# mcahny/vps

Hardware: AMD Instinct MI355X
Metric: frames/sec FuseTrack 1024x2048 (higher is better)
Workload: dtype f32-grade: f16x3 split operands (fp16 pair with scaled residual, 22 significand bits) on MFMA, f32 accumulate

## Files before the change

include/vps_hip.h:

```cpp
#ifndef VPS_HIP_H
#define VPS_HIP_H

#include <stdint.h>

#ifdef __cplusplus
extern "C" {
#endif

int vps_abi_version(void);
const char* vps_build_info(void);

enum { VPS_ACT_NONE = 0, VPS_ACT_RELU = 1, VPS_ACT_LEAKY = 2 };
enum { VPS_PREC_F32 = 0, VPS_PREC_BF16 = 1, VPS_PREC_BF16X3 = 2, VPS_PREC_BF16X6 = 3, VPS_PREC_F16X3 = 4 };

typedef struct vps_conv_desc {
    const float* in;
    int32_t N, H, W;
    int32_t in_ld;
    int32_t in_coff;
    int32_t cin_pad;
    const float* w;
    int32_t cout, cout_pad, kpad;
    int32_t KH, KW, stride;
    int32_t pad_y[2], pad_x[2];
// ... 2 lines not shown
    int32_t out_ld, out_coff;
    int32_t Qh, Qw;
    int32_t os_y, os_x;
    int32_t nclass;
    const float* scale;
    const float* shift;
    const float* res;
    int32_t res_ld, res_coff, res_shift;
    int32_t act;
    float slope;
    const float* offset;
    int32_t off_ld;
    int32_t tile_n;
    int32_t ksplit;
    float* ws;
    int32_t prec;
    const void* w_split;
    int32_t korder;
    int32_t* status;
    double* gn_stats;
    int32_t gn_cpg, gn_rep;
    int32_t* tile_counter;
    const void* w_thin;
} vps_conv_desc;

int vps_conv2d(const vps_conv_desc* d, void* stream);

typedef struct vps_tensor4 {
    float* p;
    int64_t sn, sc, sh, sw;
} vps_tensor4;

int vps_resample2d(vps_tensor4 in, vps_tensor4 flow, vps_tensor4 out,
                   int B, int C, int H, int W, void* stream);

int vps_channelnorm(vps_tensor4 in, vps_tensor4 out, int B, int C, int H, int W, void* stream);

int vps_correlation(const float* in1, int ld1, int coff1, const float* in2, int ld2, int coff2,
                    float* out, int out_ld, int out_coff,
                    int N, int H, int W, int C, int max_disp, int stride2,
                    int act, float slope, void* stream);
int vps_correlation_f16(const float* in1, int ld1, int coff1, const float* in2, int ld2, int coff2,
                        float* out, int out_ld, int out_coff, int N, int H, int W, int C,
                        int max_disp, int stride2, int act, float slope, int32_t* status, void* stream);

int vps_flow_warp(const float* in, int in_ld, int in_coff, const float* flow, int flow_ld, int flow_coff,
// ... 156 lines not shown
```

vps_amd/csrc/conv_mfma.hip:

```cpp
#include "conv_common.h"

namespace {
template <int TM, int TN, int WAVES_M, int WAVES_N, bool DEFORM>
__global__ __launch_bounds__(256, 2)
void conv_mfma_f32_kernel(const vps_conv_desc d, const int M, const int tiles_m, const int tiles_n,
                          const int ksteps_per_split) {
    constexpr int BN = WAVES_N * TN * 32;
    static_assert(WAVES_M * TM * 32 == BM, "block M tile must be 128");
    static_assert(WAVES_M * WAVES_N == 4, "4 wavefronts per block");
    constexpr int NB = BN / 32;

    __shared__ __attribute__((aligned(16))) float As[BM * LDS_LD];
    __shared__ __attribute__((aligned(16))) float Bs[BN * LDS_LD];

    const int t = threadIdx.x;
    int swz = xcd_swizzle(blockIdx.x, gridDim.x);
    int tile_n, tile_m, cls, split;
    decode_tile(d, swz, tiles_n, tiles_m, tile_n, tile_m, cls, split);

    const int py = cls / d.os_x, px = cls - py * d.os_x;
    const int pad_y = d.pad_y[py], pad_x = d.pad_x[px];
    const float* __restrict__ wcls = d.w + (size_t)cls * d.cout_pad * d.kpad;

    const int H = d.H, W = d.W, KH = d.KH, KW = d.KW, cin_pad = d.cin_pad;
// ... 710 lines not shown
            else hipLaunchKernelGGL((conv_mfma_bf16h_kernel<TM, TN, WAVES_M, WAVES_N, MODE, 2, 2>), grid, block, 0, s, d, p.tiles_m, p.tiles_n, p.chunks_per_split);
        });
        return;
    }
#define VPS_CONV_LAUNCH(KERNEL) hipLaunchKernelGGL((KERNEL), grid, block, 0, s, d, p.M, p.tiles_m, p.tiles_n, p.per_split)
    if (p.kernel == CONV_K_F32) {
        if (d.offset) VPS_CONV_LAUNCH((conv_mfma_f32_kernel<TM, TN, WAVES_M, WAVES_N, true>));
        else VPS_CONV_LAUNCH((conv_mfma_f32_kernel<TM, TN, WAVES_M, WAVES_N, false>));
        return;
    }
    const bool tapmajor = d.korder == 0 && d.KH * d.KW > 1;
    with_prec<true>(d.prec, [&](auto mode) {
        constexpr int MODE = decltype(mode)::value;
        if (d.offset) VPS_CONV_LAUNCH((conv_mfma_bf16p_kernel<TM, TN, WAVES_M, WAVES_N, MODE, false, true>));
        else if (tapmajor) VPS_CONV_LAUNCH((conv_mfma_bf16p_kernel<TM, TN, WAVES_M, WAVES_N, MODE, true>));
        else VPS_CONV_LAUNCH((conv_mfma_bf16p_kernel<TM, TN, WAVES_M, WAVES_N, MODE, false>));
    });
#undef VPS_CONV_LAUNCH
}

conv_switches conv_switches_now(const vps_conv_desc& d) {
    const auto on = [](const char* name) { const char* const e = getenv(name); return !(e && atoi(e) == 0); };
    const auto not0 = [](const char* name) { const char* const e = getenv(name); return !(e && e[0] == '0'); };
    static const bool s2_halo = not0("VPS_S2_HALO"), thin = on("VPS_THIN"), debug_occ = getenv("VPS_DEBUG_OCC") != nullptr;
    conv_switches sw = {true, true, true, true, s2_halo, thin, debug_occ};
    if (d.prec != VPS_PREC_F16X3) return sw;
    if (d.tile_n == 32) {
        if (d.cout > 16) sw.n32 = not0("VPS_N32");
        else if (d.nclass == 4) sw.n16t = on("VPS_N16T");
    } else if (d.tile_n <= 128 && d.KH == 1) sw.pw = on("VPS_PW");
    else if (d.tile_n == 128 && d.KH == 3 && d.stride == 1) sw.h8p = on("VPS_H8P");
    return sw;
}

const conv_limits& conv_limits_once(const bool debug) {
    static const conv_limits lim = [debug] {
        conv_limits l = {};
        int dev = 0;
        (void)hipGetDevice(&dev);
        (void)hipDeviceGetAttribute(&l.cus, hipDeviceAttributeMultiprocessorCount, dev);
        vpsi_conv_pw_limits(l, debug);
        vpsi_conv_thin_limits(l, debug);
        if (debug) vpsi_conv_q_debug_occ();
        return l;
    }();
    return lim;
}

}

extern "C" int vps_conv2d(const vps_conv_desc* dp, void* stream) {
    if (!dp) return VPS_EARG(1);
    const vps_conv_desc& d = *dp;
    if (const int e = vpsi_conv_check(d)) return e;
    const conv_switches sw = conv_switches_now(d);
    const conv_plan p = vpsi_conv_plan(d, conv_limits_once(sw.debug_occ), sw);
    hipStream_t s = (hipStream_t)stream;
    switch (p.kernel) {
        case CONV_K_NONE: return p.err;
        case CONV_K_SMALL3X3V: case CONV_K_SMALL_BATCHED: case CONV_K_SMALL: vpsi_launch_conv_small(d, p, s); break;
        case CONV_K_THIN: vpsi_launch_conv_thin(d, p, s); break;
        case CONV_K_DCN256:
            hipLaunchKernelGGL((conv_mfma_bf16p_kernel<2, 4, 2, 2, VPS_PREC_F16X3, false, true>), dim3(p.grid), dim3(p.block), 0, s, d, p.M, p.tiles_m, p.tiles_n, p.per_split);
            break;
        case CONV_K_N16T: case CONV_K_N32: case CONV_K_N16: vpsi_launch_conv_n16(d, p, s); break;
        case CONV_K_H8S2: vpsi_launch_conv_h8s2(d, p, s); break;
        case CONV_K_H8P: vpsi_launch_conv_h8p(d, p, s); break;
        case CONV_K_H8: vpsi_launch_conv_h8(d, p, s); break;
        case CONV_K_PW: vpsi_launch_conv_pw(d, p, s); break;
        case CONV_K_Q: vpsi_launch_conv_q(d, p, s); break;
        default:
            if (d.tile_n == 128) launch_conv<2, 2, 2, 2>(d, p, s);
            else if (d.tile_n == 64) launch_conv<2, 1, 2, 2>(d, p, s);
            else launch_conv<1, 1, 4, 1>(d, p, s);
    }
    int st = vps_launch_status();
    if (st || !p.needs_reduce) return st;
    const size_t total = (size_t)d.nclass * p.M * d.cout;
    if (p.reduce_v4) hipLaunchKernelGGL(conv_splitk_reduce_kernel<4>, dim3(stream_grid((long)(total / 4), 256)), dim3(256), 0, s, d, p.M);
    else hipLaunchKernelGGL(conv_splitk_reduce_kernel<1>, dim3(stream_grid((long)total, 256)), dim3(256), 0, s, d, p.M);
    return vps_launch_status();
}
```

vps_amd/csrc/conv_plan.cpp:

```cpp
#include "conv_plan.h"
#include <stdint.h>

namespace {

constexpr int BM = 128, BK = 32;

inline int cdiv(long a, long b) { return (int)((a + b - 1) / b); }
inline size_t in_bytes(const vps_conv_desc& d) { return (size_t)d.N * d.H * d.W * d.in_ld * sizeof(float); }
inline size_t out_bytes(const vps_conv_desc& d) { return (size_t)d.N * d.Ho * d.Wo * d.out_ld * sizeof(float); }
inline bool two_plane(int prec) { return prec == VPS_PREC_F16X3 || prec == VPS_PREC_BF16X3 || prec == VPS_PREC_BF16; }

constexpr int H8_MIN_CHUNKS = 3;
constexpr int PW_MIN_ROUNDS = 2;

conv_plan fail(conv_plan p, int n) { p.kernel = CONV_K_NONE; p.err = VPS_EARG(n); return p; }

conv_plan plan_small(const vps_conv_desc& d, conv_plan p) {
    p.block = 256;
    p.G = 1; p.logG = 0;
    while (p.G < 64 && p.G < (d.cin_pad >> 2)) { p.G <<= 1; ++p.logG; }
    const size_t wbytes = (size_t)(d.cout <= 2 ? 2 : 4) * d.kpad * sizeof(float);
    if (d.KH == 3 && d.KW == 3 && d.stride == 1 && d.nclass == 1 && d.pad_y[0] == 1 && d.pad_x[0] == 1 && d.Ho == d.H && d.Wo == d.W &&
        wbytes <= 150 * 1024 && (d.cout <= 2 || d.cout_pad >= 4) && in_bytes(d) < 0xFFFFFFF0ull &&
        (long)d.N * d.H * d.W < 0x7fffffffL) {
// ... 23 lines not shown
    long blocks = (waves + 3) / 4; if (blocks > 8192) blocks = 8192; if (blocks < 1) blocks = 1;
    p.kernel = CONV_K_SMALL; p.grid = (unsigned)blocks;
    return p;
}

bool plan_thin(const vps_conv_desc& d, const conv_limits& lim, const conv_switches& sw, conv_plan& p) {
    if (!sw.thin || !d.w_thin || d.prec != VPS_PREC_F16X3 || d.offset || d.res || d.nclass != 1 || d.ksplit != 1 || d.korder != 0) return false;
    if (d.KH != d.KW || d.cout_pad != 64 || d.tile_n != 64 || (d.cout & 3) || ((uintptr_t)d.w_thin & 15)) return false;
    if (d.pad_y[0] != d.KH / 2 || d.pad_x[0] != d.KH / 2 || d.pad_y[1] != d.KH / 2 || d.pad_x[1] != d.KH / 2) return false;
    if (in_bytes(d) >= 0xFFFFFFF0ull) return false;
    if (((d.out_ld | d.out_coff) & 3) || ((uintptr_t)d.out & 15) || out_bytes(d) >= 0xFFFFFFF0ull) return false;
    int i = 0;
    while (i < 4 && !(d.KH == conv_thin_shapes[i].ks && d.stride == conv_thin_shapes[i].s && d.cin_pad == conv_thin_shapes[i].c4)) ++i;
    if (i == 4) return false;
    const int ph = conv_thin_shapes[i].ph;
    const int tiles_x = (d.Qw + 31) / 32, tiles_y = (d.Qh + ph - 1) / ph;
    const long ntiles = (long)d.N * tiles_x * tiles_y;
    if (ntiles < 512 || ntiles > 0x7fffffffL) return false;
    const int resident = (lim.thin_per_cu[i] > 0 ? lim.thin_per_cu[i] : 1) * (lim.cus > 0 ? lim.cus : 256);
    const long rounds = (ntiles + resident - 1) / resident;
    p.kernel = CONV_K_THIN; p.thin = i; p.tiles_n = tiles_x; p.tiles_m = tiles_y; p.ntiles = (int)ntiles;
    p.grid = (unsigned)((ntiles + rounds - 1) / rounds); p.block = 256;
    return true;
}

bool plan_pw(const vps_conv_desc& d, const conv_limits& lim, const conv_switches& sw, conv_plan& p) {
    if (!sw.pw || d.prec != VPS_PREC_F16X3 || d.offset || d.KH != 1 || d.KW != 1 || d.nclass != 1 || d.ksplit != 1 || d.gn_stats) return false;
    if (d.pad_y[0] || d.pad_x[0] || (d.cin_pad & 31) || d.kpad != d.cin_pad || (d.tile_n != 128 && d.tile_n != 64)) return false;
    const int nk = d.kpad / BK;
    if (nk < 2 || (nk & 1)) return false;
    if (d.Ho != d.Qh || d.Wo != d.Qw || (d.stride == 1 && (d.H != d.Qh || d.W != d.Qw))) return false;
    if (((d.cout | d.out_ld | d.out_coff) & 3) || ((uintptr_t)d.out & 15) || out_bytes(d) >= 0xFFFFFE00ull) return false;
    if (d.res && (((d.res_ld | d.res_coff) & 3) || ((uintptr_t)d.res & 15) || d.res_shift < 0 || d.res_shift > 4 ||
                  (size_t)d.N * (d.Ho >> d.res_shift) * (d.Wo >> d.res_shift) * d.res_ld * sizeof(float) >= 0xFFFFFE00ull)) return false;
    if (in_bytes(d) >= 0xFFFFFE00ull) return false;
    const int per_cu = lim.pw_per_cu[d.tile_n == 128 ? 1 : 0];
    const int resident = (per_cu > 0 ? per_cu : 1) * (lim.cus > 0 ? lim.cus : 256);
    const long total = (long)p.tiles_m * p.tiles_n;
    const int unit = 8 * p.tiles_n;
    if (resident < unit || total < (long)PW_MIN_ROUNDS * resident) return false;
    const long rounds = (total + resident - 1) / resident;
    long grid = (total + rounds - 1) / rounds;
    grid = (grid + unit - 1) / unit * unit;
    if (grid > resident) grid = resident / unit * unit;
    const int mper = (int)(grid / unit);
    p.kernel = CONV_K_PW; p.grid = (unsigned)grid; p.nk = nk; p.nit = (p.tiles_m + mper * 8 - 1) / (mper * 8);
    return true;
}

}

const conv_thin_shape conv_thin_shapes[4] = {{8, 3, 1, 8}, {12, 3, 1, 8}, {4, 7, 2, 8}, {12, 7, 2, 4}};

const char* vpsi_conv_kernel_name(int kernel) {
    static const char* const names[] = {"none", "small3x3v", "small_batched", "small", "thin", "dcn256", "n16t", "n32", "n16",
                                        "h8s2", "h8p", "h8", "halo", "pw", "q", "f32", "bf16p"};
    return kernel >= 0 && kernel <= CONV_K_BF16P ? names[kernel] : "?";
}

int vpsi_conv_check(const vps_conv_desc& d) {
    if (!d.in || !d.out) return VPS_EARG(2);
    if (d.prec < VPS_PREC_F32 || d.prec > VPS_PREC_F16X3) return VPS_EARG(12);
    if (d.prec == VPS_PREC_F32 ? !d.w : !d.w_split) return VPS_EARG(13);
    if ((d.in_ld & 3) || (d.in_coff & 3) || (d.cin_pad & 3) || d.cin_pad <= 0) return VPS_EARG(3);
    if ((d.kpad % BK) || d.kpad < d.KH * d.KW * d.cin_pad || (d.korder != 0 && d.korder != 1)) return VPS_EARG(4);
    if (d.korder == 1 && d.kpad != d.KH * d.KW * ((d.cin_pad + BK - 1) / BK) * BK) return VPS_EARG(14);
    if (d.tile_n != 32 && d.tile_n != 64 && d.tile_n != 128 && !(d.tile_n == 256 && d.offset && d.prec == VPS_PREC_F16X3 && d.korder == 1)) return VPS_EARG(5);
    if (d.cout_pad % d.tile_n || d.cout > d.cout_pad || d.cout <= 0) return VPS_EARG(6);
    if (d.nclass != d.os_y * d.os_x || d.nclass < 1 || d.os_y > 2 || d.os_x > 2) return VPS_EARG(7);
    if (d.ksplit < 1 || (d.ksplit > 1 && !d.ws)) return VPS_EARG(8);
    if (d.offset && (d.nclass != 1 || d.off_ld < 2 * d.KH * d.KW || d.KH * d.KW > 9 || d.H > 65535 || d.W > 65535)) return VPS_EARG(9);
    if (d.offset && d.prec != VPS_PREC_F32 && d.korder != 1) return VPS_EARG(17);
    if (((uintptr_t)d.in & 15) || ((uintptr_t)d.w & 15) || ((uintptr_t)d.w_split & 15)) return VPS_EARG(10);
    if (d.prec != VPS_PREC_F32 && in_bytes(d) >= 0xFFFFFFF0ull) return VPS_EARG(16);
    if (d.gn_stats && (!d.offset || d.prec == VPS_PREC_F32 || d.ksplit != 1 || d.gn_rep < 1 || (d.gn_rep & (d.gn_rep - 1)) || (d.gn_cpg != 4 && (d.gn_cpg < 8 || (d.gn_cpg & 7))) || d.cout % d.gn_cpg ||
                       ((d.cout | d.out_ld | d.out_coff) & 3) || ((uintptr_t)d.out & 15) || d.res || ((uintptr_t)d.gn_stats & 7)))
        return VPS_EARG(15);
    const long Ml = (long)d.N * d.Qh * d.Qw;
    if (Ml <= 0 || Ml > 0x7fffffffL) return VPS_EARG(11);
    return 0;
}

conv_plan vpsi_conv_plan(const vps_conv_desc& d, const conv_limits& lim, const conv_switches& sw) {
    conv_plan p = {};
    const int M = p.M = (int)((long)d.N * d.Qh * d.Qw);
    if (d.cout <= 4 && d.prec == VPS_PREC_F32 && !d.offset && d.ksplit == 1 && d.tile_n == 32) return plan_small(d, p);
    if (plan_thin(d, lim, sw, p)) return p;

    const int BN = d.tile_n;
    const int tiles_m = p.tiles_m = cdiv(M, BM);
    const int tiles_n = p.tiles_n = d.cout_pad / BN;
    const int ksteps = d.kpad / BK;
    p.block = 256;
    p.needs_reduce = d.ksplit > 1 && !d.tile_counter;
    if (BN == 256) {
        p.per_split = cdiv(ksteps, d.ksplit);
        if (cdiv(ksteps, p.per_split) != d.ksplit) return fail(p, 20);
        p.kernel = CONV_K_DCN256; p.grid = (unsigned)((long)tiles_m * tiles_n * d.ksplit); p.reduce_v4 = true;
        return p;
    }
    const int ntap = d.KH * d.KW;
    const int nch = d.korder == 1 ? ksteps / ntap : 0;
    const bool chunk_split = d.ksplit > 1 && d.korder == 1 && nch > 0 && cdiv(nch, cdiv(nch, d.ksplit)) == d.ksplit;
    const int per_split = p.per_split = chunk_split ? cdiv(nch, d.ksplit) * ntap : cdiv(ksteps, d.ksplit);
    p.chunks_per_split = per_split / ntap;
    if (cdiv(ksteps, per_split) != d.ksplit) return fail(p, 20);
    const long nblk = (long)tiles_m * tiles_n * d.nclass * d.ksplit;
    if (nblk <= 0 || nblk > 0x7fffffffL) return fail(p, 21);
    p.reduce_v4 = !((d.cout | d.cout_pad | d.out_ld | d.out_coff) & 3) && !((uintptr_t)d.out & 15) &&
                  (!d.res || (!((d.res_ld | d.res_coff) & 3) && !((uintptr_t)d.res & 15)));
// ... 39 lines not shown
```

vps_amd/csrc/conv_plan.h:

```cpp
#pragma once
#include <stddef.h>
#include "../../include/vps_hip.h"

#ifndef VPS_EARG
#define VPS_EARG(x) (-1000 - (x))
#endif

enum conv_kernel {
    CONV_K_NONE = 0,
    CONV_K_SMALL3X3V,
    CONV_K_SMALL_BATCHED,
    CONV_K_SMALL,
    CONV_K_THIN,
    CONV_K_DCN256,
    CONV_K_N16T,
    CONV_K_N32,
    CONV_K_N16,
    CONV_K_H8S2,
    CONV_K_H8P,
    CONV_K_H8,
    CONV_K_HALO,
    CONV_K_PW,
    CONV_K_Q,
    CONV_K_F32,
    CONV_K_BF16P,
};

struct conv_plan {
    int kernel;
    int err;
    int M;
    int tiles_m, tiles_n;
    int per_split;
    int chunks_per_split;
    unsigned grid, block;
    size_t smem;
    int nk, nit;
    int G, logG, nslot;
    int runs_per_row, total_runs;
    int thin;
    int ntiles;
    bool needs_reduce;
    bool reduce_v4;
};

struct conv_limits {
    int cus;
    int pw_per_cu[2];
    int thin_per_cu[4];
};

struct conv_switches {
    bool pw;
    bool h8p;
    bool n16t;
    bool n32;
    bool s2_halo;
    bool thin;
    bool debug_occ;
};

struct conv_thin_shape { int c4, ks, s, ph; };
extern const conv_thin_shape conv_thin_shapes[4];

int vpsi_conv_check(const vps_conv_desc& d);
conv_plan vpsi_conv_plan(const vps_conv_desc& d, const conv_limits& lim, const conv_switches& sw);
const char* vpsi_conv_kernel_name(int kernel);

#ifdef __HIPCC__
void vpsi_launch_conv_small(const vps_conv_desc& d, const conv_plan& p, hipStream_t s);
void vpsi_launch_conv_thin(const vps_conv_desc& d, const conv_plan& p, hipStream_t s);
void vpsi_launch_conv_n16(const vps_conv_desc& d, const conv_plan& p, hipStream_t s);
void vpsi_launch_conv_h8(const vps_conv_desc& d, const conv_plan& p, hipStream_t s);
void vpsi_launch_conv_h8p(const vps_conv_desc& d, const conv_plan& p, hipStream_t s);
void vpsi_launch_conv_h8s2(const vps_conv_desc& d, const conv_plan& p, hipStream_t s);
void vpsi_launch_conv_pw(const vps_conv_desc& d, const conv_plan& p, hipStream_t s);
void vpsi_launch_conv_q(const vps_conv_desc& d, const conv_plan& p, hipStream_t s);
void vpsi_conv_pw_limits(conv_limits& lim, bool debug);
void vpsi_conv_thin_limits(conv_limits& lim, bool debug);
void vpsi_conv_q_debug_occ();
#endif
```

vps_amd/csrc/info.hip:

```cpp
#include "common.h"

#define VPS_ABI_VERSION 19

extern "C" int vps_abi_version(void) { return VPS_ABI_VERSION; }

extern "C" const char* vps_build_info(void) {
#define VPS_STR2(x) #x
#define VPS_STR(x) VPS_STR2(x)
    return "libvpship abi=" VPS_STR(VPS_ABI_VERSION) " arch=gfx950 wave=64 mfma=f32_32x32x2,bf16_32x32x16(split x3/x6),f16_32x32x16(split x3) "
           "kernels=conv_mfma,flow_ops,nn_ops,det_ops,head_ops,pan_ops,post_ops,jpeg_ops";
}
```

vps_amd/flownet2.py:

```python
import torch
import torch.nn as nn

from . import hip, nhwc
from .base import HipModule


def _conv(cin, cout, k=3, stride=1):
    return nn.Sequential(nn.Conv2d(cin, cout, k, stride=stride, padding=(k - 1) // 2, bias=True), nn.LeakyReLU(0.1))


def _iconv(cin, cout):
    return nn.Sequential(nn.Conv2d(cin, cout, 3, padding=1, bias=True))


def _deconv(cin, cout):
    return nn.Sequential(nn.ConvTranspose2d(cin, cout, 4, 2, 1, bias=True), nn.LeakyReLU(0.1))


def _pred(cin):
    return nn.Conv2d(cin, 2, 3, padding=1, bias=True)


class _Net(nn.Module):

# ... 113 lines not shown
        self.conv1 = _conv(64, 64, stride=2); self.conv1_1 = _conv(64, 128)
        self.conv2 = _conv(128, 128, stride=2); self.conv2_1 = _conv(128, 128)
        self.conv3 = _conv(128, 256, stride=2); self.conv3_1 = _conv(256, 256)
        self.conv4 = _conv(256, 512, stride=2); self.conv4_1 = _conv(512, 512)
        self.conv5 = _conv(512, 512, stride=2); self.conv5_1 = _conv(512, 512)
        self.conv6 = _conv(512, 1024, stride=2); self.conv6_1 = _conv(1024, 1024)
        self.deconv5 = _deconv(1024, 512); self.deconv4 = _deconv(1026, 256)
        self.deconv3 = _deconv(770, 128); self.deconv2 = _deconv(386, 64)
        self.inter_conv5 = _iconv(1026, 512); self.inter_conv4 = _iconv(770, 256)
        self.inter_conv3 = _iconv(386, 128); self.inter_conv2 = _iconv(194, 64)
        self.predict_flow6 = _pred(1024); self.predict_flow5 = _pred(512); self.predict_flow4 = _pred(256)
        self.predict_flow3 = _pred(128); self.predict_flow2 = _pred(64)
        for n in ('6_to_5', '5_to_4', '4_to_3', '3_to_2'):
            setattr(self, 'upsampled_flow' + n, nn.ConvTranspose2d(2, 2, 4, 2, 1))

    def run(self, x6, ws, tag):
        p = self._p
        N, H, W = x6.N, x6.H, x6.W
        h2, w2 = H // 4, W // 4
        cat2 = ws.fmap(tag + 'cat2', N, h2, w2, 194)
        cat3 = ws.fmap(tag + 'cat3', N, h2 // 2, w2 // 2, 386)
        cat4 = ws.fmap(tag + 'cat4', N, h2 // 4, w2 // 4, 770)
        cat5 = ws.fmap(tag + 'cat5', N, h2 // 8, w2 // 8, 1026)
        c0 = p['conv0'](x6.window(0, 6), ws=ws, name=tag + 'c0', temp=True)
        t = p['conv1'](c0, ws=ws, name=tag + 'c1', temp=True)
        ws.release(c0)
        c1 = p['conv1_1'](t, ws=ws, name=tag + 'c11', temp=True)
        ws.release(t)
        t = p['conv2'](c1, ws=ws, name=tag + 'c2', temp=True)
        ws.release(c1)
        p['conv2_1'](t, out=cat2.window(0, 128), ws=ws)
        ws.release(t)
        t = p['conv3'](cat2.window(0, 128), ws=ws, name=tag + 'c3', temp=True)
        p['conv3_1'](t, out=cat3.window(0, 256), ws=ws)
        t = p['conv4'](cat3.window(0, 256), ws=ws, name=tag + 'c4', temp=True)
        p['conv4_1'](t, out=cat4.window(0, 512), ws=ws)
        t = p['conv5'](cat4.window(0, 512), ws=ws, name=tag + 'c5', temp=True)
        p['conv5_1'](t, out=cat5.window(0, 512), ws=ws)
        t = p['conv6'](cat5.window(0, 512), ws=ws, name=tag + 'c6', temp=True)
        c6 = p['conv6_1'](t, ws=ws, name=tag + 'c61', temp=True)
        flow = p['predict_flow6'](c6, ws=ws, name=tag + 'flow6')
        feat = c6
        for lvl, cat, enc_c, dec_c in ((5, cat5, 512, 512), (4, cat4, 512, 256), (3, cat3, 256, 128), (2, cat2, 128, 64)):
            p['upsampled_flow%d_to_%d' % (lvl + 1, lvl)](flow, out=cat.window(enc_c + dec_c, 2), ws=ws)
            p['deconv%d' % lvl](feat, out=cat.window(enc_c, dec_c), ws=ws)
            inter = p['inter_conv%d' % lvl](cat, ws=ws, name='%sinter%d' % (tag, lvl), temp=True)
            flow = p['predict_flow%d' % lvl](inter, ws=ws, name='%sflow%d' % (tag, lvl))
            ws.release(inter)
            feat = cat
        return flow


class FlowNetFusion(_Net):
    def __init__(self):
        super().__init__()
        self.conv0 = _conv(11, 64)
        self.conv1 = _conv(64, 64, stride=2); self.conv1_1 = _conv(64, 128)
        self.conv2 = _conv(128, 128, stride=2); self.conv2_1 = _conv(128, 128)
        self.deconv1 = _deconv(128, 32); self.deconv0 = _deconv(162, 16)
        self.inter_conv1 = _iconv(162, 32); self.inter_conv0 = _iconv(82, 16)
        self.predict_flow2 = _pred(128); self.predict_flow1 = _pred(32); self.predict_flow0 = _pred(16)
        self.upsampled_flow2_to_1 = nn.ConvTranspose2d(2, 2, 4, 2, 1)
        self.upsampled_flow1_to_0 = nn.ConvTranspose2d(2, 2, 4, 2, 1)

    def run(self, x11, ws, tag):
        p = self._p
        N, H, W = x11.N, x11.H, x11.W
        cat0 = ws.fmap(tag + 'cat0', N, H, W, 82)
        cat1 = ws.fmap(tag + 'cat1', N, H // 2, W // 2, 162)
        p['conv0'](x11, out=cat0.window(0, 64), ws=ws)
        t = p['conv1'](cat0.window(0, 64), ws=ws, name=tag + 'c1', temp=True)
        p['conv1_1'](t, out=cat1.window(0, 128), ws=ws)
        ws.release(t)
        t = p['conv2'](cat1.window(0, 128), ws=ws, name=tag + 'c2', temp=True)
        c2 = p['conv2_1'](t, ws=ws, name=tag + 'c21', temp=True)
        ws.release(t)
        flow2 = p['predict_flow2'](c2, ws=ws, name=tag + 'flow2')
        p['upsampled_flow2_to_1'](flow2, out=cat1.window(160, 2), ws=ws)
        p['deconv1'](c2, out=cat1.window(128, 32), ws=ws)
        ws.release(c2)
        inter1 = p['inter_conv1'](cat1, ws=ws, name=tag + 'inter1', temp=True)
        flow1 = p['predict_flow1'](inter1, ws=ws, name=tag + 'flow1')
        ws.release(inter1)
        p['upsampled_flow1_to_0'](flow1, out=cat0.window(80, 2), ws=ws)
        p['deconv0'](cat1, out=cat0.window(64, 16), ws=ws)
        inter0 = p['inter_conv0'](cat0, ws=ws, name=tag + 'inter0', temp=True)
        return p['predict_flow0'](inter0, ws=ws, name=tag + 'flow0', keep=True)


class FlowNet2(HipModule):

    def __init__(self, args=None, batchNorm=False, div_flow=20., requires_grad=False):
        super().__init__()
        assert not batchNorm
# ... 82 lines not shown
```

vps_amd/hip.py:

```python
import ctypes
import os
from ctypes import (POINTER, Structure, byref, c_char_p, c_double, c_float, c_int, c_int32, c_int64, c_uint64,
                    c_void_p)

import torch

_HERE = os.path.dirname(os.path.abspath(__file__))
LIB_PATH = os.environ.get('VPS_HIP_LIB') or os.path.join(_HERE, 'csrc', 'libvpship.so')
ABI_VERSION = 19

ACT_NONE, ACT_RELU, ACT_LEAKY = 0, 1, 2
PREC_F32, PREC_BF16, PREC_BF16X3, PREC_BF16X6, PREC_F16X3 = 0, 1, 2, 3, 4

SYMBOLS = [
    'vps_abi_version', 'vps_build_info', 'vps_conv2d', 'vps_resample2d', 'vps_channelnorm', 'vps_correlation',
    'vps_flow_warp', 'vps_nchw_to_nhwc', 'vps_nhwc_to_nchw', 'vps_resize', 'vps_pool3x3s2', 'vps_bfp_gather',
    'vps_bfp_scatter', 'vps_bfp_scatter_all', 'vps_axpb', 'vps_flow_prep', 'vps_flow_prep_pad', 'vps_flow_stage', 'vps_flow_stage_full', 'vps_groupnorm_relu', 'vps_groupnorm_apply', 'vps_tcea_temporal',
    'vps_tcea_modulate', 'vps_tcea_modulate_ld', 'vps_correlation_f16', 'vps_roi_align', 'vps_nms_batched', 'vps_delta2bbox', 'vps_bbox_overlaps',
    'vps_row_softmax', 'vps_mask_count', 'vps_mask_commit', 'vps_mask_removal', 'vps_mask_removal_dep', 'vps_mask_removal_hist', 'vps_frame_tail', 'vps_mask_level', 'vps_panoptic_combine',
    'vps_panoptic_combine_dev', 'vps_rpn_select', 'vps_rpn_collect', 'vps_maskroi_select', 'vps_maskroi_finish', 'vps_track_assign', 'vps_pan_instances',
    'vps_unify_hist', 'vps_unify_tables', 'vps_unify_write', 'vps_image_prep', 'vps_resize_u8', 'vps_segment_stats', 'vps_segment_paint', 'vps_pair_count',
    'vps_png_info', 'vps_png_decode_bgr8', 'vps_jpeg_info', 'vps_jpeg_decode_coef', 'vps_jpeg_reconstruct',
]


class ConvDesc(Structure):
    _fields_ = [
        ('inp', c_void_p), ('N', c_int32), ('H', c_int32), ('W', c_int32),
        ('in_ld', c_int32), ('in_coff', c_int32), ('cin_pad', c_int32),
        ('w', c_void_p), ('cout', c_int32), ('cout_pad', c_int32), ('kpad', c_int32),
        ('KH', c_int32), ('KW', c_int32), ('stride', c_int32),
        ('pad_y', c_int32 * 2), ('pad_x', c_int32 * 2),
        ('out', c_void_p), ('Ho', c_int32), ('Wo', c_int32), ('out_ld', c_int32), ('out_coff', c_int32),
        ('Qh', c_int32), ('Qw', c_int32), ('os_y', c_int32), ('os_x', c_int32), ('nclass', c_int32),
        ('scale', c_void_p), ('shift', c_void_p), ('res', c_void_p),
        ('res_ld', c_int32), ('res_coff', c_int32), ('res_shift', c_int32),
        ('act', c_int32), ('slope', c_float),
        ('offset', c_void_p), ('off_ld', c_int32),
        ('tile_n', c_int32), ('ksplit', c_int32), ('ws', c_void_p),
        ('prec', c_int32), ('w_split', c_void_p), ('korder', c_int32), ('status', c_void_p),
        ('gn_stats', c_void_p), ('gn_cpg', c_int32), ('gn_rep', c_int32), ('tile_counter', c_void_p), ('w_thin', c_void_p),
    ]


class Tensor4(Structure):
    _fields_ = [('p', c_void_p), ('sn', c_int64), ('sc', c_int64), ('sh', c_int64), ('sw', c_int64)]


class PanInst(Structure):
    _fields_ = [('sx0', c_int32), ('sy0', c_int32), ('sx1', c_int32), ('sy1', c_int32), ('seg_ch', c_int32),
                ('bx1', c_int32), ('by1', c_int32), ('bx2', c_int32), ('by2', c_int32), ('mask_idx', c_int32)]


_lib = None
_host = None


class VpsHipError(RuntimeError):
    pass


def csrc_sha16():
    import glob
    import hashlib
# ... 166 lines not shown
```

vps_amd/nhwc.py:

```python
import ctypes
import math
import os
import weakref
from ctypes import c_float, c_int, c_void_p

import torch

from . import hip


def _ceil(a, b):
    return (a + b - 1) // b * b


_PREC_NAMES = {'f32': hip.PREC_F32, 'bf16': hip.PREC_BF16, 'bf16x3': hip.PREC_BF16X3, 'bf16x6': hip.PREC_BF16X6, 'f16x3': hip.PREC_F16X3}
PREC_NAMES = _PREC_NAMES
_PLANES = {hip.PREC_BF16: 1, hip.PREC_BF16X3: 2, hip.PREC_BF16X6: 3, hip.PREC_F16X3: 3}
MFMA_PRODUCTS = {hip.PREC_F32: 1, hip.PREC_BF16: 1, hip.PREC_BF16X3: 3, hip.PREC_BF16X6: 6, hip.PREC_F16X3: 3}
F16_SLOTS = 4096
_F16_STATUS = {}
_F16_LAYERS = {}
_F16_NEXT = [1]
F16_FALLBACKS = [0]

# ... 491 lines not shown
                               '%d->%d k%dx%d s%d %s%s n%d %dx%d tile%d ksplit%d p%d' % (self.cin, self.cout, self.KH, self.KW, self.stride,
                                                                                   'T' if self.transposed else '', 'D' if self.deform else '',
                                                                                   x.N, x.H, x.W, tile_n, ksplit, self.prec),
                               self.bytes(x.N, x.H, x.W, res is not None)))
        else:
            hip.conv2d(d)
        if len(cache) >= 16:
            cache.clear()
        cache[ckey] = (d, wsb if ksplit > 1 else None, x.t, out.t, None if res is None else res.t, None if offset is None else offset.t)
        return out

    def bytes(self, x_N, x_H, x_W, has_res=False):
        Ho, Wo = self.out_hw(x_H, x_W)
        wbytes = self.nclass * self.cout * self.KH * self.KW * self.cin * (4 if self.prec == hip.PREC_F32 else 2 * _PLANES[self.prec])
        return 4.0 * x_N * (x_H * x_W * self.cin + Ho * Wo * self.cout * (2 if has_res else 1)) + wbytes

    def flops(self, x_N, x_H, x_W):
        if self.transposed:
            return 2.0 * x_N * x_H * x_W * 4 * self.cout * self.cin * self.KH * self.KW
        Ho, Wo = self.out_hw(x_H, x_W)
        return 2.0 * x_N * Ho * Wo * self.cout * self.cin * self.KH * self.KW


def pack_conv_module(m, bn=None, act=hip.ACT_NONE, slope=0.1, device='cuda', deform=False, prec=None):
    import torch.nn as nn
    bnd = None
    if bn is not None:
        bnd = dict(weight=bn.weight, bias=bn.bias, running_mean=bn.running_mean, running_var=bn.running_var, eps=bn.eps)
    if isinstance(m, nn.ConvTranspose2d):
        return PackedConv(m.weight, m.bias, bnd, stride=m.stride[0], padding=m.padding[0], act=act, slope=slope,
                          transposed=True, device=device, prec=prec)
    return PackedConv(m.weight, m.bias, bnd, stride=m.stride[0], padding=m.padding[0], act=act, slope=slope,
                      device=device, deform=deform, prec=prec)


def pack_linear(weight, bias, act=hip.ACT_NONE, device='cuda', chw=None, prec=None):
    w = weight.detach().float().cpu()
    if chw is not None:
        C, S = chw
        w = w.view(w.shape[0], C, S).permute(0, 2, 1).reshape(w.shape[0], C * S)
    return PackedConv(w.view(w.shape[0], w.shape[1], 1, 1), bias, None, 1, 0, act=act, device=device, prec=prec)


def resize(x, out, mode='bilinear', alpha=1.0):
    hip.check(hip.load().vps_resize(x.ptr(), x.ld, x.coff, x.H, x.W, out.ptr(), out.ld, out.coff, out.H, out.W,
                                    x.N, x.C, 0 if mode == 'bilinear' else 1, float(alpha), hip.stream_ptr()), 'vps_resize')
# ... 113 lines not shown
```

Baseline: 55.57.

## Fuse thin stride-1 conv0 into following stride-2 conv1 front kernel

```diff
diff --git a/include/vps_hip.h b/include/vps_hip.h
--- a/include/vps_hip.h
+++ b/include/vps_hip.h
@@ -48,6 +48,16 @@
     int32_t gn_cpg, gn_rep;
     int32_t* tile_counter;
     const void* w_thin;
+    const float* pre_in;
+    int32_t pre_in_ld, pre_in_coff, pre_cin_pad;
+    const void* pre_w_thin;
+    const float* pre_scale;
+    const float* pre_shift;
+    int32_t pre_act;
+    float pre_slope;
+    float* pre_out;
+    int32_t pre_out_ld, pre_out_coff;
+    int32_t* pre_status;
 } vps_conv_desc;
 
 int vps_conv2d(const vps_conv_desc* d, void* stream);
diff --git a/vps_amd/csrc/conv_front.hip b/vps_amd/csrc/conv_front.hip
--- /dev/null
+++ b/vps_amd/csrc/conv_front.hip
@@ -0,0 +1,254 @@
+#include "conv_common.h"
+
+namespace {
+
+constexpr int TMODE = VPS_PREC_F16X3;
+typedef _Float16 h16;
+typedef vec8<h16> h16x8;
+typedef vec4<h16> h16x4;
+
+struct FTap { int ph, j, i, idx; };
+constexpr FTap front_tap(int ts) {
+    int base = 0;
+    for (int ph = 0; ph < 4; ++ph) {
+        const int a = ph >> 1, b = ph & 1, J = 2 - a, I = 2 - b;
+        if (ts < base + J * I) {
+            const int t = ts - base, j = t / I, i = t - j * I;
+            return FTap{ph, j, i, (2 * j + a) * 3 + 2 * i + b};
+        }
+        base += J * I;
+    }
+    return FTap{0, 0, 0, 0};
+}
+template <int N, typename F>
+__device__ __forceinline__ void static_for(F&& f) {
+    if constexpr (N > 0) {
+        static_for<N - 1>(f);
+        f(std::integral_constant<int, N - 1>{});
+    }
+}
+
+template <int C4>
+struct FrontShape {
+    static constexpr int PH = 4, PW = 32;
+    static constexpr int TR = 2 * PH + 1, TC = 2 * PW + 1;
+    static constexpr int TPOS = TR * TC, NGRP = (TPOS + 31) / 32;
+    static constexpr int PR = TR + 2, PC = TC + 2, NPOS = PR * PC;
+    static constexpr int NV = C4 / 4;
+    static constexpr int NK16 = (3 * C4 + 15) / 16;
+    static constexpr int APLANE = NPOS * C4 + 16;
+    static constexpr int TWH = 3 * 2 * NK16 * 512;
+    static constexpr int SW = PW + 1;
+    static constexpr int TROWS = (2 * (PH + 1) + 2 * PH) * SW;
+    static constexpr int TPLANE = TROWS * LDS_LDH;
+    static constexpr int WBH = 8 * 512;
+    static constexpr size_t smem = (size_t)(2 * APLANE + TWH + 2 * TPLANE + 2 * WBH) * 2 + 128 * sizeof(float);
+    static_assert((2 * APLANE) % 8 == 0 && TWH % 8 == 0 && (2 * TPLANE) % 8 == 0, "16-byte aligned regions");
+    static_assert(smem <= 160 * 1024, "LDS budget of the CU");
+};
+
+template <int C4, bool STORE>
+__global__ __launch_bounds__(512, 1)
+void conv_front_kernel(const vps_conv_desc d, const int tiles_x, const int tiles_y) {
+    typedef FrontShape<C4> S;
+    typedef Split<TMODE> SM;
+    constexpr int PH = S::PH, PW = S::PW, TC = S::TC, TPOS = S::TPOS, NGRP = S::NGRP, PC = S::PC, NPOS = S::NPOS, NV = S::NV, NK16 = S::NK16;
+    constexpr int APLANE = S::APLANE, TWH = S::TWH, SW = S::SW, TPLANE = S::TPLANE, WBH = S::WBH;
+    constexpr int NLOAD = (NPOS * NV + 511) / 512;
+    constexpr int NTW = (TWH / 8 + 511) / 512;
+    extern __shared__ __attribute__((aligned(16))) unsigned char front_smem[];
+    h16* const As = reinterpret_cast<h16*>(front_smem);
+    h16* const Tw = As + 2 * APLANE;
+    h16* const Ts = Tw + TWH;
+    h16* const Wb = Ts + 2 * TPLANE;
+    float* const scsh = reinterpret_cast<float*>(Wb + 2 * WBH);
+
+    const int t = threadIdx.x, lane = t & 63;
+    const int wave = __builtin_amdgcn_readfirstlane(t >> 6);
+    const int p32 = lane & 31, kh = lane >> 5;
+    const int wm = wave >> 1, wn = wave & 1;
+    const int tile = xcd_swizzle(blockIdx.x, gridDim.x);
+    const int tx = tile % tiles_x, tq = tile / tiles_x;
+    const int ty = tq % tiles_y, n = tq / tiles_y;
+    const int H0 = d.H, W0 = d.W;
+    const int y0 = ty * 2 * PH - 1, x0 = tx * 2 * PW - 1;
+
+    const __amdgpu_buffer_rsrc_t in_rsrc = make_rsrc(d.pre_in, (unsigned)((size_t)d.N * H0 * W0 * d.pre_in_ld * sizeof(float)));
+    const __amdgpu_buffer_rsrc_t po_rsrc = make_rsrc(d.pre_out, STORE ? (unsigned)((size_t)d.N * H0 * W0 * d.pre_out_ld * sizeof(float)) : 0u);
+    const u32x4* __restrict__ twg = reinterpret_cast<const u32x4*>(d.pre_w_thin);
+    const u32x4* __restrict__ w1g = reinterpret_cast<const u32x4*>(d.w_split);
+    constexpr int KST = 36, WPLANE16 = 2 * KST * 64;
+
+    f32x4 v[NLOAD];
+#pragma unroll
+    for (int i = 0; i < NLOAD; ++i) {
+        const int idx = t + i * 512;
+        const int pos = idx / NV, q = idx - pos * NV;
+        const int r = pos / PC, c = pos - r * PC;
+        const int iy = y0 - 1 + r, ix = x0 - 1 + c;
+        const bool ok = idx < NPOS * NV && iy >= 0 && iy < H0 && ix >= 0 && ix < W0;
+        const unsigned off = (unsigned)((((size_t)n * H0 + iy) * W0 + ix) * d.pre_in_ld + d.pre_in_coff + 4 * q) * 4u;
+        v[i] = buffer_load16<f32x4>(in_rsrc, ok ? off : 0xFFFFFFF0u, 0);
+    }
+    u32x4 twreg[NTW];
+    auto load_tw = [&](const int b) {
+#pragma unroll
+        for (int u = 0; u < NTW; ++u) {
+            const int i = min(t + u * 512, TWH / 8 - 1);
+            twreg[u] = twg[((i >> 6) * 2 + b) * 64 + (i & 63)];
+        }
+    };
+    auto store_tw = [&]() {
+#pragma unroll
+        for (int u = 0; u < NTW; ++u)
+            if (t + u * 512 < TWH / 8) reinterpret_cast<u32x4*>(Tw)[t + u * 512] = twreg[u];
+    };
+    auto load_w1 = [&](const int step) {
+        const int f = t >> 6, pl = f >> 2, m = (f >> 1) & 1, nb = f & 1;
+        return w1g[pl * WPLANE16 + (nb * KST + 2 * step + m) * 64 + lane];
+    };
+    load_tw(0);
+    u32x4 w1reg = load_w1(front_tap(0).idx);
+
+    if (t < 128) {
+        const int c = t & 63;
+        float val = t < 64 ? 1.f : 0.f;
+        if (t < 64 && d.pre_scale) val = d.pre_scale[c];
+        if (t >= 64 && d.pre_shift) val = d.pre_shift[c];
+        scsh[t] = val;
+    }
+    if (t < 8) {
+        const h16x4 z = {(h16)0, (h16)0, (h16)0, (h16)0};
+        *reinterpret_cast<h16x4*>(&As[(t >> 2) * APLANE + NPOS * C4 + (t & 3) * 4]) = z;
+    }
+    float amax0 = 0.f, amax1 = 0.f;
+#pragma unroll
+    for (int i = 0; i < NLOAD; ++i) {
+        const int idx = t + i * 512;
+        h16x4 pl[SM::NSA];
+        split_act<TMODE>(v[i], pl, amax0);
+        if (idx < NPOS * NV) {
+#pragma unroll
+            for (int p = 0; p < 2; ++p) *reinterpret_cast<h16x4*>(&As[p * APLANE + idx * 4]) = pl[p];
+        }
+    }
+    store_tw();
+    reinterpret_cast<u32x4*>(Wb)[t] = w1reg;
+    __syncthreads();
+
+    const float ns = d.pre_act == VPS_ACT_RELU ? 0.f : (d.pre_act == VPS_ACT_LEAKY ? d.pre_slope : 1.f);
+    f32x16 acc[1][1];
+#pragma unroll
+    for (int r = 0; r < 16; ++r) acc[0][0][r] = 0.f;
+
+    for (int chunk = 0; chunk < 2; ++chunk) {
+        if (chunk == 1) {
+            store_tw();
+            __syncthreads();
+        }
+        for (int g = wave; g < NGRP; g += 8) {
+            const int P = g * 32 + p32;
+            const int Pc = min(P, TPOS - 1);
+            const int r = Pc / TC, c = Pc - r * TC;
+            f32x16 pa;
+#pragma unroll
+            for (int e = 0; e < 16; ++e) pa[e] = 0.f;
+#pragma unroll
+            for (int j = 0; j < 3; ++j) {
+#pragma unroll
+                for (int s = 0; s < NK16; ++s) {
+                    h16x8 af[2], wf[3];
+                    const int base = ((r + j) * PC + c) * C4 + s * 16 + kh * 8;
+#pragma unroll
+                    for (int p = 0; p < 2; ++p) {
+                        const h16x4 lo = *reinterpret_cast<const h16x4*>(&As[p * APLANE + base]);
+                        const h16x4 hi = *reinterpret_cast<const h16x4*>(&As[p * APLANE + base + 4]);
+                        af[p] = __builtin_shufflevector(lo, hi, 0, 1, 2, 3, 4, 5, 6, 7);
+                        wf[p] = *reinterpret_cast<const h16x8*>(&Tw[((j * 2 + p) * NK16 + s) * 512 + lane * 8]);
+                    }
+                    wf[2] = derive_weight_plane<TMODE>(wf[0]);
+#pragma unroll
+                    for (int q = 0; q < SM::NT; ++q) pa = split_mfma<TMODE>(wf[SM::PB[q]], af[SM::PA[q]], pa);
+                }
+            }
+            const int y = y0 + r, x = x0 + c;
+            const bool inside = P < TPOS && y >= 0 && y < H0 && x >= 0 && x < W0;
+            const bool own = STORE && inside && r >= 1 && c >= 1;
+            const unsigned pixoff = (unsigned)((((size_t)n * H0 + y) * W0 + x) * d.pre_out_ld + d.pre_out_coff + 32 * chunk + 4 * kh) * 4u;
+            const int ph = (r & 1) * 2 + (c & 1);
+            const int row = (ph * (PH + 1) - (ph == 3 ? 1 : 0)) * SW + (r >> 1) * SW + (c >> 1);
+#pragma unroll
+            for (int gq = 0; gq < 4; ++gq) {
+                const int co = 32 * chunk + 8 * gq + 4 * kh;
+                const f32x4 sc = *reinterpret_cast<const f32x4*>(&scsh[co]);
+                const f32x4 sh = *reinterpret_cast<const f32x4*>(&scsh[64 + co]);
+                f32x4 o;
+#pragma unroll
+                for (int e = 0; e < 4; ++e) {
+                    const float tt = pa[4 * gq + e] * sc[e] + sh[e];
+                    o[e] = fmaxf(tt, 0.f) + ns * fminf(tt, 0.f);
+                }
+                if constexpr (STORE)
+                    __builtin_amdgcn_raw_buffer_store_b128(__builtin_bit_cast(u32x4, o), po_rsrc, (int)(own ? pixoff + (unsigned)(8 * gq) * 4u : 0xFFFFFFF0u), 0, 0);
+                if (!inside) o = f32x4{0.f, 0.f, 0.f, 0.f};
+                h16x4 pl[SM::NSA];
+                split_act<TMODE>(o, pl, amax1);
+                if (P < TPOS) {
+#pragma unroll
+                    for (int p = 0; p < 2; ++p)
+                        *reinterpret_cast<h16x4*>(&Ts[p * TPLANE + row * LDS_LDH + ((gq ^ lds_swz(row)) << 3) + (kh << 2)]) = pl[p];
+                }
+            }
+        }
+        if (chunk == 0) load_tw(1);
+        __syncthreads();
+
+        static_for<9>([&](auto ts_tag) {
+            constexpr int TS = decltype(ts_tag)::value;
+            constexpr FTap tp = front_tap(TS);
+            constexpr FTap nx = front_tap((TS + 1) % 9);
+            const int step = chunk * 9 + TS;
+            const int bb = step & 1;
+            const bool more = TS + 1 < 9 || chunk == 0;
+            if (more) w1reg = load_w1((TS + 1 < 9 ? chunk : 1) * 9 + nx.idx);
+            constexpr int phrow = (tp.ph * (PH + 1) - (tp.ph == 3 ? 1 : 0)) * SW;
+            const int hrow = phrow + (wm + tp.j) * SW + p32 + tp.i;
+            h16x8 af[2][2], wf[2][3];
+#pragma unroll
+            for (int m = 0; m < 2; ++m) {
+                const int off = hrow * LDS_LDH + (((2 * m + kh) ^ lds_swz(hrow)) << 3);
+#pragma unroll
+                for (int p = 0; p < 2; ++p) {
+                    af[m][p] = *reinterpret_cast<const h16x8*>(&Ts[p * TPLANE + off]);
+                    wf[m][p] = *reinterpret_cast<const h16x8*>(&Wb[bb * WBH + ((p * 2 + m) * 2 + wn) * 512 + lane * 8]);
+                }
+                wf[m][2] = derive_weight_plane<TMODE>(wf[m][0]);
+            }
+#pragma unroll
+            for (int m = 0; m < 2; ++m)
+#pragma unroll
+                for (int q = 0; q < SM::NT; ++q) acc[0][0] = split_mfma<TMODE>(wf[m][SM::PB[q]], af[m][SM::PA[q]], acc[0][0]);
+            if (more) reinterpret_cast<u32x4*>(Wb)[(bb ^ 1) * (WBH / 8) + t] = w1reg;
+            __syncthreads();
+        });
+    }
+    report_range<TMODE>(d, amax1);
+    if (d.pre_status && !(amax0 <= 65504.f)) atomicOr(d.pre_status, 1);
+    conv_epilogue<1, 1, 64, true, 5, false, false, 2, false>(d, acc, 0, tile, 0, 0, 0, 0, 0, wm, wn, lane, tile);
+}
+
+template <int C4, bool STORE>
+void launch_front(const vps_conv_desc& d, const conv_plan& p, hipStream_t s) {
+    static const int raised = (int)hipFuncSetAttribute(reinterpret_cast<const void*>(&conv_front_kernel<C4, STORE>),
+                                                       hipFuncAttributeMaxDynamicSharedMemorySize, (int)FrontShape<C4>::smem);
+    (void)raised;
+    hipLaunchKernelGGL((conv_front_kernel<C4, STORE>), dim3(p.grid), dim3(p.block), FrontShape<C4>::smem, s, d, p.tiles_n, p.tiles_m);
+}
+
+}
+
+__attribute__((visibility("hidden")))
+void vpsi_launch_conv_front(const vps_conv_desc& d, const conv_plan& p, hipStream_t s) {
+    if (d.pre_cin_pad == 8) { if (d.pre_out) launch_front<8, true>(d, p, s); else launch_front<8, false>(d, p, s); }
+    else { if (d.pre_out) launch_front<12, true>(d, p, s); else launch_front<12, false>(d, p, s); }
+}
diff --git a/vps_amd/csrc/conv_mfma.hip b/vps_amd/csrc/conv_mfma.hip
--- a/vps_amd/csrc/conv_mfma.hip
+++ b/vps_amd/csrc/conv_mfma.hip
@@ -756,9 +756,11 @@
 conv_switches conv_switches_now(const vps_conv_desc& d) {
     const auto on = [](const char* name) { const char* const e = getenv(name); return !(e && atoi(e) == 0); };
     const auto not0 = [](const char* name) { const char* const e = getenv(name); return !(e && e[0] == '0'); };
+    const auto front_default = [](const char* name) { const char* const e = getenv(name); return e ? atoi(e) != 0 : CONV_FRONT_DEFAULT; };
     static const bool s2_halo = not0("VPS_S2_HALO"), thin = on("VPS_THIN"), debug_occ = getenv("VPS_DEBUG_OCC") != nullptr;
-    conv_switches sw = {true, true, true, true, s2_halo, thin, debug_occ};
+    conv_switches sw = {true, true, true, true, s2_halo, thin, debug_occ, false};
     if (d.prec != VPS_PREC_F16X3) return sw;
+    if (d.pre_in) sw.front = front_default("VPS_FRONT_FUSE");
     if (d.tile_n == 32) {
         if (d.cout > 16) sw.n32 = not0("VPS_N32");
         else if (d.nclass == 4) sw.n16t = on("VPS_N16T");
@@ -794,6 +796,7 @@
         case CONV_K_NONE: return p.err;
         case CONV_K_SMALL3X3V: case CONV_K_SMALL_BATCHED: case CONV_K_SMALL: vpsi_launch_conv_small(d, p, s); break;
         case CONV_K_THIN: vpsi_launch_conv_thin(d, p, s); break;
+        case CONV_K_FRONT: vpsi_launch_conv_front(d, p, s); break;
         case CONV_K_DCN256:
             hipLaunchKernelGGL((conv_mfma_bf16p_kernel<2, 4, 2, 2, VPS_PREC_F16X3, false, true>), dim3(p.grid), dim3(p.block), 0, s, d, p.M, p.tiles_m, p.tiles_n, p.per_split);
             break;
diff --git a/vps_amd/csrc/conv_plan.cpp b/vps_amd/csrc/conv_plan.cpp
--- a/vps_amd/csrc/conv_plan.cpp
+++ b/vps_amd/csrc/conv_plan.cpp
@@ -69,6 +69,20 @@
     p.kernel = CONV_K_THIN; p.thin = i; p.tiles_n = tiles_x; p.tiles_m = tiles_y; p.ntiles = (int)ntiles;
     p.grid = (unsigned)((ntiles + rounds - 1) / rounds); p.block = 256;
     return true;
+}
+
+bool front_shape(const vps_conv_desc& d) {
+    if (d.prec != VPS_PREC_F16X3 || d.offset || d.res || d.gn_stats || d.nclass != 1 || d.ksplit != 1 || d.korder != 1) return false;
+    if (d.KH != 3 || d.KW != 3 || d.stride != 2 || d.cin_pad != 64 || d.cout != 64 || d.cout_pad != 64 || d.tile_n != 64 || d.kpad != 576) return false;
+    if (d.pad_y[0] != 1 || d.pad_x[0] != 1 || d.Qh != d.Ho || d.Qw != d.Wo || d.Ho != (d.H - 1) / 2 + 1 || d.Wo != (d.W - 1) / 2 + 1) return false;
+    if ((d.pre_cin_pad != 8 && d.pre_cin_pad != 12) || !d.pre_w_thin || ((uintptr_t)d.pre_w_thin & 15) || ((uintptr_t)d.pre_in & 15)) return false;
+    if ((d.pre_in_ld & 3) || (d.pre_in_coff & 3) || d.pre_in_coff < 0 || d.pre_in_coff + d.pre_cin_pad > d.pre_in_ld) return false;
+    if ((size_t)d.N * d.H * d.W * d.pre_in_ld * sizeof(float) >= 0xFFFFFFF0ull) return false;
+    if (d.pre_out && (((d.pre_out_ld | d.pre_out_coff) & 3) || ((uintptr_t)d.pre_out & 15) || d.pre_out_coff < 0 || d.pre_out_coff + 64 > d.pre_out_ld ||
+                      (size_t)d.N * d.H * d.W * d.pre_out_ld * sizeof(float) >= 0xFFFFFFF0ull)) return false;
+    const long thin_tiles = (long)d.N * ((d.W + 31) / 32) * ((d.H + 7) / 8), t8 = (long)d.N * ((d.Qh + 7) / 8) * ((d.Qw + 31) / 32);
+    if (thin_tiles < 512 || t8 < 256 || t8 * 256 * 2 > (long)d.N * d.Qh * d.Qw * 3) return false;
+    return (long)d.N * ((d.Qh + 3) / 4) * ((d.Qw + 31) / 32) <= 0x7fffffffL;
 }
 
 bool plan_pw(const vps_conv_desc& d, const conv_limits& lim, const conv_switches& sw, conv_plan& p) {
@@ -100,13 +114,14 @@
 const conv_thin_shape conv_thin_shapes[4] = {{8, 3, 1, 8}, {12, 3, 1, 8}, {4, 7, 2, 8}, {12, 7, 2, 4}};
 
 const char* vpsi_conv_kernel_name(int kernel) {
-    static const char* const names[] = {"none", "small3x3v", "small_batched", "small", "thin", "dcn256", "n16t", "n32", "n16",
+    static const char* const names[] = {"none", "small3x3v", "small_batched", "small", "thin", "front", "dcn256", "n16t", "n32", "n16",
                                         "h8s2", "h8p", "h8", "halo", "pw", "q", "f32", "bf16p"};
     return kernel >= 0 && kernel <= CONV_K_BF16P ? names[kernel] : "?";
 }
 
 int vpsi_conv_check(const vps_conv_desc& d) {
-    if (!d.in || !d.out) return VPS_EARG(2);
+    if ((!d.in && !d.pre_in) || !d.out) return VPS_EARG(2);
+    if (d.pre_in && !front_shape(d)) return VPS_EARG(18);
     if (d.prec < VPS_PREC_F32 || d.prec > VPS_PREC_F16X3) return VPS_EARG(12);
     if (d.prec == VPS_PREC_F32 ? !d.w : !d.w_split) return VPS_EARG(13);
     if ((d.in_ld & 3) || (d.in_coff & 3) || (d.cin_pad & 3) || d.cin_pad <= 0) return VPS_EARG(3);
@@ -133,6 +148,12 @@
     const int M = p.M = (int)((long)d.N * d.Qh * d.Qw);
     if (d.cout <= 4 && d.prec == VPS_PREC_F32 && !d.offset && d.ksplit == 1 && d.tile_n == 32) return plan_small(d, p);
     if (plan_thin(d, lim, sw, p)) return p;
+    if (d.pre_in) {
+        if (!sw.front) return fail(p, 22);
+        p.kernel = CONV_K_FRONT; p.tiles_n = (d.Qw + 31) / 32; p.tiles_m = (d.Qh + 3) / 4;
+        p.ntiles = d.N * p.tiles_m * p.tiles_n; p.grid = (unsigned)p.ntiles; p.block = 512;
+        return p;
+    }
 
     const int BN = d.tile_n;
     const int tiles_m = p.tiles_m = cdiv(M, BM);
diff --git a/vps_amd/csrc/conv_plan.h b/vps_amd/csrc/conv_plan.h
--- a/vps_amd/csrc/conv_plan.h
+++ b/vps_amd/csrc/conv_plan.h
@@ -12,6 +12,7 @@
     CONV_K_SMALL_BATCHED,
     CONV_K_SMALL,
     CONV_K_THIN,
+    CONV_K_FRONT,
     CONV_K_DCN256,
     CONV_K_N16T,
     CONV_K_N32,
@@ -58,7 +59,10 @@
     bool s2_halo;
     bool thin;
     bool debug_occ;
+    bool front;
 };
+
+constexpr bool CONV_FRONT_DEFAULT = true;
 
 struct conv_thin_shape { int c4, ks, s, ph; };
 extern const conv_thin_shape conv_thin_shapes[4];
@@ -70,6 +74,7 @@
 #ifdef __HIPCC__
 void vpsi_launch_conv_small(const vps_conv_desc& d, const conv_plan& p, hipStream_t s);
 void vpsi_launch_conv_thin(const vps_conv_desc& d, const conv_plan& p, hipStream_t s);
+void vpsi_launch_conv_front(const vps_conv_desc& d, const conv_plan& p, hipStream_t s);
 void vpsi_launch_conv_n16(const vps_conv_desc& d, const conv_plan& p, hipStream_t s);
 void vpsi_launch_conv_h8(const vps_conv_desc& d, const conv_plan& p, hipStream_t s);
 void vpsi_launch_conv_h8p(const vps_conv_desc& d, const conv_plan& p, hipStream_t s);
diff --git a/vps_amd/csrc/info.hip b/vps_amd/csrc/info.hip
--- a/vps_amd/csrc/info.hip
+++ b/vps_amd/csrc/info.hip
@@ -1,6 +1,6 @@
 #include "common.h"
 
-#define VPS_ABI_VERSION 19
+#define VPS_ABI_VERSION 20
 
 extern "C" int vps_abi_version(void) { return VPS_ABI_VERSION; }
 
diff --git a/vps_amd/flownet2.py b/vps_amd/flownet2.py
--- a/vps_amd/flownet2.py
+++ b/vps_amd/flownet2.py
@@ -159,9 +159,7 @@
         cat3 = ws.fmap(tag + 'cat3', N, h2 // 2, w2 // 2, 386)
         cat4 = ws.fmap(tag + 'cat4', N, h2 // 4, w2 // 4, 770)
         cat5 = ws.fmap(tag + 'cat5', N, h2 // 8, w2 // 8, 1026)
-        c0 = p['conv0'](x6.window(0, 6), ws=ws, name=tag + 'c0', temp=True)
-        t = p['conv1'](c0, ws=ws, name=tag + 'c1', temp=True)
-        ws.release(c0)
+        t = nhwc.conv_front(p['conv0'], p['conv1'], x6.window(0, 6), ws=ws, name=tag + 'c1', temp=True)
         c1 = p['conv1_1'](t, ws=ws, name=tag + 'c11', temp=True)
         ws.release(t)
         t = p['conv2'](c1, ws=ws, name=tag + 'c2', temp=True)
@@ -205,8 +203,7 @@
         N, H, W = x11.N, x11.H, x11.W
         cat0 = ws.fmap(tag + 'cat0', N, H, W, 82)
         cat1 = ws.fmap(tag + 'cat1', N, H // 2, W // 2, 162)
-        p['conv0'](x11, out=cat0.window(0, 64), ws=ws)
-        t = p['conv1'](cat0.window(0, 64), ws=ws, name=tag + 'c1', temp=True)
+        t = nhwc.conv_front(p['conv0'], p['conv1'], x11, store=cat0.window(0, 64), ws=ws, name=tag + 'c1', temp=True)
         p['conv1_1'](t, out=cat1.window(0, 128), ws=ws)
         ws.release(t)
         t = p['conv2'](cat1.window(0, 128), ws=ws, name=tag + 'c2', temp=True)
diff --git a/vps_amd/hip.py b/vps_amd/hip.py
--- a/vps_amd/hip.py
+++ b/vps_amd/hip.py
@@ -7,7 +7,7 @@
 
 _HERE = os.path.dirname(os.path.abspath(__file__))
 LIB_PATH = os.environ.get('VPS_HIP_LIB') or os.path.join(_HERE, 'csrc', 'libvpship.so')
-ABI_VERSION = 19
+ABI_VERSION = 20
 
 ACT_NONE, ACT_RELU, ACT_LEAKY = 0, 1, 2
 PREC_F32, PREC_BF16, PREC_BF16X3, PREC_BF16X6, PREC_F16X3 = 0, 1, 2, 3, 4
@@ -40,6 +40,9 @@
         ('tile_n', c_int32), ('ksplit', c_int32), ('ws', c_void_p),
         ('prec', c_int32), ('w_split', c_void_p), ('korder', c_int32), ('status', c_void_p),
         ('gn_stats', c_void_p), ('gn_cpg', c_int32), ('gn_rep', c_int32), ('tile_counter', c_void_p), ('w_thin', c_void_p),
+        ('pre_in', c_void_p), ('pre_in_ld', c_int32), ('pre_in_coff', c_int32), ('pre_cin_pad', c_int32), ('pre_w_thin', c_void_p),
+        ('pre_scale', c_void_p), ('pre_shift', c_void_p), ('pre_act', c_int32), ('pre_slope', c_float),
+        ('pre_out', c_void_p), ('pre_out_ld', c_int32), ('pre_out_coff', c_int32), ('pre_status', c_void_p),
     ]
 
 
diff --git a/vps_amd/nhwc.py b/vps_amd/nhwc.py
--- a/vps_amd/nhwc.py
+++ b/vps_amd/nhwc.py
@@ -537,6 +537,86 @@
         return 2.0 * x_N * Ho * Wo * self.cout * self.cin * self.KH * self.KW
 
 
+FRONT_FUSE_DEFAULT = 1
+
+
+def front_fuse_level():
+    e = os.environ.get('VPS_FRONT_FUSE')
+    try:
+        return FRONT_FUSE_DEFAULT if e is None else int(e)
+    except ValueError:
+        return 0
+
+
+def _front_size_ok(N, H, W):
+    Ho, Wo = (H - 1) // 2 + 1, (W - 1) // 2 + 1
+    t8 = N * ((Ho + 7) // 8) * ((Wo + 31) // 32)
+    return N * ((W + 31) // 32) * ((H + 7) // 8) >= 512 and t8 >= 256 and t8 * 512 <= N * Ho * Wo * 3
+
+
+def conv_front(pre, conv, x, store=None, ws=None, name=None, temp=False):
+    fused = (front_fuse_level() >= (1 if store is None else 2) and pre.prec == hip.PREC_F16X3 and conv.prec == hip.PREC_F16X3 and getattr(pre, 'w_thin', None) is not None
+             and (pre.KH, pre.KW, pre.stride, pre.pad_y[0], pre.cout, pre.nclass) == (3, 3, 1, 1, 64, 1) and pre.cin_pad in (8, 12)
+             and (conv.KH, conv.KW, conv.stride, conv.pad_y[0], conv.cin, conv.cout, conv.korder, conv.nclass) == (3, 3, 2, 1, 64, 64, 1, 1)
+             and not pre.deform and not conv.deform
+             and (store is None or not ((store.ld | store.coff) & 3)) and _front_size_ok(x.N, x.H, x.W))
+    if not fused:
+        mid = pre(x, ws=ws, name=name + '.pre', temp=True) if store is None else pre(x, out=store, ws=ws)
+        out = conv(mid, ws=ws, name=name, temp=temp)
+        if store is None:
+            ws.release(mid)
+        return out
+    assert x.C >= pre.cin and x.C <= pre.cin_pad and x.coff % 4 == 0 and x.ld % 4 == 0 and x.coff + pre.cin_pad <= x.ld, (x.C, x.coff, x.ld)
+    assert store is None or ((store.N, store.H, store.W, store.C) == (x.N, x.H, x.W, 64) and store.t.device == x.t.device)
+    Ho, Wo = conv.out_hw(x.H, x.W)
+    out = ws.fmap(name, x.N, Ho, Wo, 64, temp=temp)
+    ckey = ('front', id(pre), x.t.data_ptr(), x.N, x.H, x.W, x.ld, x.coff, out.t.data_ptr(), out.ld, out.coff,
+            None if store is None else (store.t.data_ptr(), store.ld, store.coff), getattr(hip.stream_ptr(), 'value', None) or 0)
+    cache = conv.__dict__.setdefault('_dcache', {})
+    hit = cache.get(ckey)
+    if hit is not None and CONV_TRACE is None:
+        hip.conv2d(hit[0])
+        return out
+    d = hip.ConvDesc()
+    d.N, d.H, d.W = x.N, x.H, x.W
+    d.in_ld, d.in_coff, d.cin_pad = 64, 0, 64
+    d.prec, d.korder = conv.prec, conv.korder
+    d.w_split = conv.w_split.data_ptr()
+    d.cout, d.cout_pad, d.kpad = conv.cout, conv.cout_pad, conv.kpad
+    d.KH, d.KW, d.stride = 3, 3, 2
+    d.pad_y[0], d.pad_y[1] = conv.pad_y; d.pad_x[0], d.pad_x[1] = conv.pad_x
+    d.out = out.t.data_ptr(); d.Ho, d.Wo, d.out_ld, d.out_coff = Ho, Wo, out.ld, out.coff
+    d.Qh, d.Qw, d.os_y, d.os_x, d.nclass = Ho, Wo, 1, 1, 1
+    d.scale = conv.scale.data_ptr() if conv.scale is not None else None
+    d.shift = conv.shift.data_ptr() if conv.shift is not None else None
+    d.act, d.slope = conv.act, conv.slope
+    d.tile_n, d.ksplit = conv.tile_n, 1
+    st = f16_status(x.t.device).data_ptr()
+    d.status = st + 4 * getattr(conv, 'f16_slot', 0)
+    d.pre_in = x.t.data_ptr(); d.pre_in_ld, d.pre_in_coff, d.pre_cin_pad = x.ld, x.coff, pre.cin_pad
+    d.pre_w_thin = pre.w_thin.data_ptr()
+    d.pre_scale = pre.scale.data_ptr() if pre.scale is not None else None
+    d.pre_shift = pre.shift.data_ptr() if pre.shift is not None else None
+    d.pre_act, d.pre_slope = pre.act, pre.slope
+    if store is not None:
+        d.pre_out = store.t.data_ptr(); d.pre_out_ld, d.pre_out_coff = store.ld, store.coff
+    d.pre_status = st + 4 * getattr(pre, 'f16_slot', 0)
+    if CONV_TRACE is not None:
+        e0 = torch.cuda.Event(enable_timing=True); e1 = torch.cuda.Event(enable_timing=True)
+        e0.record()
+        hip.conv2d(d)
+        e1.record()
+        CONV_TRACE.append((pre.flops(x.N, x.H, x.W) + conv.flops(x.N, x.H, x.W), e0, e1,
+                           '%d->64->64 front k3x3 s1+s2 n%d %dx%d tile64 ksplit1 p%d' % (pre.cin, x.N, x.H, x.W, conv.prec),
+                           4.0 * x.N * (x.H * x.W * (pre.cin + (64 if store is not None else 0)) + Ho * Wo * 64)))
+    else:
+        hip.conv2d(d)
+    if len(cache) >= 16:
+        cache.clear()
+    cache[ckey] = (d, None, x.t, out.t, None if store is None else store.t, pre)
+    return out
+
+
 def pack_conv_module(m, bn=None, act=hip.ACT_NONE, slope=0.1, device='cuda', deform=False, prec=None):
     import torch.nn as nn
     bnd = None
```

After: 56.06 (median of 6 runs). About the same (+0.9%).
